# danielbrathwaite/OpenGL-Path-Tracing

Measured on AMD Instinct MI355X. Metric: Mrays/sec + ms/frame @1920×1080, 8 bounces, 1/2/4/8 MI355X, higher is better.
Workload: dtype f32

## Files before the change

### opengl-path-tracing_amd/csrc/pt_cull.h

```cpp
#pragma once

#include "pt_math.h"

namespace ptc {

constexpr float kWindowLo = 0.0001f * 0x1.ff8p-1f;
constexpr float kWindowRay = 0x1.4p-20f;

PT_HD float min_t(float tf, float t) {
#if defined(__HIP_DEVICE_COMPILE__)
    return __builtin_amdgcn_fmed3f(tf, t, -__builtin_huge_valf());
#else
    return fminf(tf, t);
#endif
}

PT_HD void cull_addends(pt::f3 o, pt::f3 rd, const float cm[3], const float ws[3], pt::f3& ol, pt::f3& oh) {
    const pt::f3 ord = pt::mk(-(o.x * rd.x), -(o.y * rd.y), -(o.z * rd.z));
    const float ax = __builtin_fabsf(rd.x), ay = __builtin_fabsf(rd.y), az = __builtin_fabsf(rd.z);
    const pt::f3 e = pt::mk(__builtin_fmaf(cm[0], ax, 0x1p-17f * __builtin_fabsf(ord.x)),
                            __builtin_fmaf(cm[1], ay, 0x1p-17f * __builtin_fabsf(ord.y)),
                            __builtin_fmaf(cm[2], az, 0x1p-17f * __builtin_fabsf(ord.z)));
    const float omax = fmaxf(fmaxf(__builtin_fabsf(o.x), __builtin_fabsf(o.y)), __builtin_fabsf(o.z));
    const float wx = __builtin_fmaf(kWindowRay, omax, ws[0]), wy = __builtin_fmaf(kWindowRay, omax, ws[1]),
                wz = __builtin_fmaf(kWindowRay, omax, ws[2]);
    ol = ord - e;
    oh = ord + pt::mk(__builtin_fmaf(wx, ax, e.x), __builtin_fmaf(wy, ay, e.y), __builtin_fmaf(wz, az, e.z));
}

PT_HD bool cull_hit(float nx, float fx, float ny, float fy, float nz, float fz, pt::f3 rd, pt::f3 ol, pt::f3 oh,
                    float cur_t, float c_lo) {
    const float xn = __builtin_fmaf(nx, rd.x, ol.x), xf = __builtin_fmaf(fx, rd.x, oh.x);
    const float yn = __builtin_fmaf(ny, rd.y, ol.y), yf = __builtin_fmaf(fy, rd.y, oh.y);
    const float zn = __builtin_fmaf(nz, rd.z, ol.z), zf = __builtin_fmaf(fz, rd.z, oh.z);
    const float tn = fmaxf(fmaxf(xn, yn), zn);
    const float tf = fminf(fminf(xf, yf), zf);
    return fmaxf(tn, c_lo) <= min_t(tf, cur_t);
}

inline bool window_slack(const float* bvh, int n_nodes, const float* tris, float ws[3]) {
    const double u = 0x1p-24;
    const float inf = __builtin_huge_valf();
    ws[0] = ws[1] = ws[2] = 0.0f;
    if (n_nodes <= 0) return true;
    double M2 = 0.0;
    for (int q = 0; q < 3; q++) {
        const double m = fmax(fabs((double)bvh[q]), fabs((double)bvh[4 + q]));
        M2 += m * m;
    }
    M2 = sqrt(M2);
    double worst[3] = {0.0, 0.0, 0.0};
    for (int i = 0; i < n_nodes; i++) {
        const float* nd = bvh + 12 * (size_t)i;
        if (!(nd[8] > -1.0f)) continue;
        for (int k = 0; k < 2; k++) {
            const float* t = tris + 16 * (size_t)(int)nd[8 + k];
            const pt::f3 v0 = pt::mk(t[0], t[1], t[2]), v1 = pt::mk(t[4], t[5], t[6]), v2 = pt::mk(t[8], t[9], t[10]);
            const pt::f3 n = pt::normalize(pt::cross(v1 - v0, v2 - v0));
            const float d0 = -pt::dot(n, v0);
            if (!(fabs((double)n.x) + fabs((double)n.y) + fabs((double)n.z) < (double)inf)) continue;
            const double V[3][3] = {{v0.x, v0.y, v0.z}, {v1.x, v1.y, v1.z}, {v2.x, v2.y, v2.z}};
            const double nn[3] = {n.x, n.y, n.z};
            double E1[3], E2[3], L2 = 0.0, rho = 0.0;
            for (int q = 0; q < 3; q++) { E1[q] = V[1][q] - V[0][q]; E2[q] = V[2][q] - V[0][q]; }
            const double N[3] = {E1[1] * E2[2] - E2[1] * E1[2], E1[2] * E2[0] - E2[2] * E1[0], E1[0] * E2[1] - E2[0] * E1[1]};
            const double D = nn[0] * N[0] + nn[1] * N[1] + nn[2] * N[2];
            for (int a = 0; a < 3; a++) {
                const int b = (a + 1) % 3;
                double l2 = 0.0;
                for (int q = 0; q < 3; q++) l2 += (V[b][q] - V[a][q]) * (V[b][q] - V[a][q]);
                L2 = fmax(L2, l2);
                rho = fmax(rho, fabs(nn[0] * V[a][0] + nn[1] * V[a][1] + nn[2] * V[a][2] + (double)d0));
            }
            const double L = sqrt(L2);
            if (!(D > 0.0) || !(L2 <= 0x1p14 * D) || !(rho <= L)) return false;
            const double kappa = L2 / D, z = 1.06 * 0x1p-140 * L / D;
            const double sigma_t = u * (7.2 * M2 + 4.4 * fabs((double)d0)) + 1.14 * rho + 6.5 * z;
            for (int q = 0; q < 3; q++) {
                const double ext = fmax(fmax(V[0][q], V[1][q]), V[2][q]) - fmin(fmin(V[0][q], V[1][q]), V[2][q]);
                worst[q] = fmax(worst[q], 21.4 * u * kappa * ext + 1.021 * sigma_t + 2.0 * z);
            }
        }
    }
    for (int q = 0; q < 3; q++)
        if (!(worst[q] < 0x1p60)) return false;
    for (int q = 0; q < 3; q++) ws[q] = nextafterf((float)(1.25 * worst[q] * (1.0 + 0x1p-20)), inf);
    return true;
}

struct SweepRay { pt::f3 rp, rn, ol, oh; };
PT_HD SweepRay sweep_ray(pt::f3 rd, pt::f3 ol, pt::f3 oh) {
    SweepRay r;
    r.rp = pt::mk(rd.x > 0.0f ? rd.x : 0.0f, rd.y > 0.0f ? rd.y : 0.0f, rd.z > 0.0f ? rd.z : 0.0f);
    r.rn = pt::mk(rd.x > 0.0f ? 0.0f : rd.x, rd.y > 0.0f ? 0.0f : rd.y, rd.z > 0.0f ? 0.0f : rd.z);
    r.ol = ol;
    r.oh = oh;
    return r;
}
PT_HD bool sweep_hit(float lx, float hx, float ly, float hy, float lz, float hz, const SweepRay& r, float t0, float c_lo) {
    const float xn = __builtin_fmaf(lx, r.rp.x, __builtin_fmaf(hx, r.rn.x, r.ol.x));
    const float xf = __builtin_fmaf(hx, r.rp.x, __builtin_fmaf(lx, r.rn.x, r.oh.x));
    const float yn = __builtin_fmaf(ly, r.rp.y, __builtin_fmaf(hy, r.rn.y, r.ol.y));
    const float yf = __builtin_fmaf(hy, r.rp.y, __builtin_fmaf(ly, r.rn.y, r.oh.y));
    const float zn = __builtin_fmaf(lz, r.rp.z, __builtin_fmaf(hz, r.rn.z, r.ol.z));
    const float zf = __builtin_fmaf(hz, r.rp.z, __builtin_fmaf(lz, r.rn.z, r.oh.z));
    const float tn = fmaxf(fmaxf(xn, yn), zn);
    const float tf = fminf(fminf(xf, yf), zf);
    return fmaxf(tn, c_lo) <= min_t(tf, t0);
}
PT_HD unsigned sweep_push(unsigned m, bool hit) {
#if defined(__HIP_DEVICE_COMPILE__) && !defined(PT_SWEEP_NO_ADDC)
    unsigned r;
    const unsigned long long c = __builtin_amdgcn_ballot_w64(hit);
    unsigned long long co;
    asm("v_addc_co_u32 %0, %1, %2, %2, %3" : "=v"(r), "=s"(co) : "v"(m), "s"(c));
    return r;
#else
    return m + m + (hit ? 1u : 0u);
#endif
}
template <class T>
PT_HD unsigned sweep_mask(const SweepRay& r, float t0, float c_lo, T table, int n) {
    unsigned m = 0u;
    for (int k = n - 1; k >= 0; k--) {
        const auto a = table[2 * k], b = table[2 * k + 1];
        m = sweep_push(m, sweep_hit(a.x, a.y, a.z, a.w, b.x, b.y, r, t0, c_lo));
    }
    return m;
}
#if defined(__clang__)
#define PT_SWEEP_UNROLL _Pragma("unroll")
#else
#define PT_SWEEP_UNROLL
#endif
PT_HD void sweep_issue_fence() {
#if defined(__HIP_DEVICE_COMPILE__)
    __builtin_amdgcn_sched_barrier(0);
#endif
}
template <int D> struct SweepChunk { float q[D][6]; };
template <int D, class T>
PT_HD void sweep_chunk_load(SweepChunk<D>& c, T table, int k) {
    PT_SWEEP_UNROLL
    for (int j = 0; j < D; j++) {
        const auto a = table[2 * (k - j)], b = table[2 * (k - j) + 1];
        c.q[j][0] = a.x, c.q[j][1] = a.y, c.q[j][2] = a.z, c.q[j][3] = a.w, c.q[j][4] = b.x, c.q[j][5] = b.y;
    }
}
template <int D>
PT_HD unsigned sweep_chunk_test(unsigned m, const SweepChunk<D>& c, const SweepRay& r, float t0, float c_lo) {
    PT_SWEEP_UNROLL
    for (int j = 0; j < D; j++)
        m = sweep_push(m, sweep_hit(c.q[j][0], c.q[j][1], c.q[j][2], c.q[j][3], c.q[j][4], c.q[j][5], r, t0, c_lo));
    return m;
}
template <int D, class T>
PT_HD unsigned sweep_mask_piped(const SweepRay& r, float t0, float c_lo, T table, int n) {
    static_assert(D >= 1 && D <= 8, "boxes in flight");
    unsigned m = 0u;
    int k = n - 1;
    for (int j = n % D; j > 0; j--, k--) {
        const auto a = table[2 * k], b = table[2 * k + 1];
        m = sweep_push(m, sweep_hit(a.x, a.y, a.z, a.w, b.x, b.y, r, t0, c_lo));
    }
    if (k < 0) return m;
    SweepChunk<D> ca, cb;
    sweep_chunk_load(ca, table, k);
    for (; k >= 3 * D - 1; k -= 2 * D) {
        sweep_chunk_load(cb, table, k - D);
        sweep_issue_fence();
        m = sweep_chunk_test(m, ca, r, t0, c_lo);
        sweep_chunk_load(ca, table, k - 2 * D);
        sweep_issue_fence();
        m = sweep_chunk_test(m, cb, r, t0, c_lo);
    }
    if (k >= 2 * D - 1) {
        sweep_chunk_load(cb, table, k - D);
        m = sweep_chunk_test(m, ca, r, t0, c_lo);
        return sweep_chunk_test(m, cb, r, t0, c_lo);
    }
    return sweep_chunk_test(m, ca, r, t0, c_lo);
}
template <class T>
PT_HD unsigned sweep_mask(pt::f3 rd, pt::f3 ol, pt::f3 oh, float t0, float c_lo, T table, int n) {
    return sweep_mask(sweep_ray(rd, ol, oh), t0, c_lo, table, n);
}
PT_HD bool sweep_root_hit(const float box[6], const SweepRay& r, float t0, float c_lo) {
    return sweep_hit(box[0], box[1], box[2], box[3], box[4], box[5], r, t0, c_lo);
}

}
```

### opengl-path-tracing_amd/csrc/pt_launch_plan.cpp

```cpp
#include "pt_launch_plan.h"

#include "pt_pool.h"

#include "../../include/pt_api.h"

#include <algorithm>
#include <cmath>

namespace ptl {

static int resident_waves(int minw, bool lds) { return minw ? minw : (lds ? 7 : 6); }

static bool lds_staged(const SceneFacts& f, const Tuning& t, const Image& im, const State& s) {
    if (t.variant == 3) return false;
    if (f.lds_bytes <= kLdsSceneSmall) return true;
    return !s.counting && !t.minw && im.rpp == 1 && f.lds_bytes <= kLdsSceneMax;
}

bool cons_walk_on(const SceneFacts& f, const Tuning& t, bool counting) {
    if (!f.walk_nested || t.cons_off || counting) return false;
    const size_t mw = (size_t)resident_waves(t.minw, true);
    const auto blocks = [mw](size_t b) { return b ? std::min(mw, kLdsCu / b) : mw; };
    return blocks(f.lds_bytes_sk) >= blocks(f.lds_bytes);
}

bool window_cull_on(const SceneFacts& f, const Tuning& t, int flags, bool counting) {
    return cons_walk_on(f, t, counting) && !t.win_off && !f.win_bad && !(flags & PT_FLAG_MOLLER_TRUMBORE);
}

bool sweep_on(const SceneFacts& f, const Tuning& t, bool counting) {
    return cons_walk_on(f, t, counting) && f.sweep_ok && !t.sweep_off;
}

static bool wide_walk_on(const SceneFacts& f, const Tuning& t, bool counting) {
    return f.wide_ok && f.scene_fast && !t.wide_off && !counting && t.minw != 8;
}

static int lds_threads(const Tuning& t, const Image& im, const State& s, size_t lds) {
    if (s.counting || t.minw || im.rpp > 1 || !lds) return 256;
    const int per_cu = (int)(kLdsCu / lds);
    int best_k = 1, best = 0;
    for (int k = 1; k <= 4; k++) {
        const int waves = std::min(per_cu, 7 / k) * k;
        if (waves > best) { best = waves; best_k = k; }
    }
    return 256 * best_k;
}

static int plan_group(const SceneFacts& f, const Tuning& t, const Image& im, const State& s, int n_frames) {
    if (t.group_force > 0) return std::min(t.group_force, n_frames);
    const bool lds_scene = lds_staged(f, t, im, s);
    const double lanes = (double)im.n_cu * 4.0 * resident_waves(t.minw, lds_scene) * 64.0;
    const double px = s.adaptive ? (double)im.n_tiles * 64.0 : (double)im.rows_local * im.width;
    const double F = px * n_frames / lanes;
    int g = (int)(std::sqrt(F) * (lds_scene ? 0.416 : 0.19) + 0.5);
    g = std::max(1, std::min(g, lds_scene ? 16 : 4));
    return std::min(g, n_frames);
}

static bool split_mode(const Tuning& t, const State& s, int n_frames, int group) {
    if (s.moments) return true;
    if (group < n_frames) return true;
    return t.group_force == 0 && n_frames <= kShortLaunch;
}

unsigned long long id_limit(const Tuning& t, const Image& im) {
    const unsigned long long pb = (unsigned long long)std::max(256, t.pull_batch);
    const unsigned long long slack = (unsigned long long)im.persist_blocks * 4ull * 2ull * pb;
    return (1ull << 32) - slack - (1ull << 20);
}

int launch_frames(const SceneFacts& f, const Tuning& t, const Image& im, const State& s, int n_frames) {
    const unsigned long long px = (unsigned long long)std::max(im.rows_local, 1) * (unsigned long long)im.width;
    const unsigned long long tiles64 = (unsigned long long)std::max(im.n_tiles, 1) * 64ull;
    const unsigned long long lim = id_limit(t, im);
    int n = n_frames;
    for (;;) {
        const int g = plan_group(f, t, im, s, n);
        if (!split_mode(t, s, n, g)) return n;
        const unsigned long long by_budget = std::max(1ull, (unsigned long long)t.scratch_budget / (px * 12ull));
        const unsigned long long ng = (unsigned long long)((n + g - 1) / g);
        const unsigned long long by_ids = (lim / tiles64) * (unsigned long long)g;
        if (((unsigned long long)n <= by_budget && ng * tiles64 < lim) || n == 1) return n;
        const unsigned long long m = std::min<unsigned long long>({(unsigned long long)n - 1, by_budget, by_ids});
        n = (int)std::max<unsigned long long>(m, 1ull);
    }
}

static KernelKey kernel_key(bool counting, bool lds, bool wide, bool split, int mw, int rpp, int nt, int walk_np) {
    const bool multi = rpp > 1;
    if (wide) {
        if (multi) return {false, false, 6, true, split, false, 256, true};
        if (nt == 512 || nt == 768) return {false, false, 6, false, split, false, nt, true};
        if (nt == 1024) return {false, false, 4, false, split, false, 1024, true};
        return {false, false, mw == 5 || mw == 7 ? mw : 6, false, split, false, 256, true};
    }
    if (nt == 512 || nt == 768) return {false, true, 6, false, split, false, nt, false};
    if (nt > 256) return {false, true, 4, false, split, false, 1024, false};
    if (counting) return {true, lds, 5, multi, split, false, 256, false};
    if (split && mw == 8 && !multi) return {false, lds, 8, false, true, false, 256, false};
    if (split && mw == 7 && !multi) return {false, lds, 7, false, true, lds && walk_np == kPadNodes, 256, false};
    return {false, lds, mw >= 6 ? 6 : 5, multi, split, false, 256, false};
}

static bool common_launch(const SceneFacts& f, const Tuning& t, const Image& im, const LaunchPlan& p) {
    if (t.common_off || t.win_off || f.win_bad || !(p.key == kCommonKey)) return false;
    if (t.minw || t.leaf_thresh || t.shade_thresh || t.trav_floor || im.tile_shift != 0 || !p.cons_walk) return false;
    if (im.flags != 0) return false;
    return f.n_spheres == 1 && f.scene_fast != 0 && f.walk_nested && f.root_child >= 0;
}

LaunchPlan plan_launch(const SceneFacts& f, const Tuning& t, const Image& im, const State& s, int n_frames,
                       bool graph) {
    LaunchPlan p{};
    const bool lds_scene = lds_staged(f, t, im, s);
    p.lds = t.variant == 0 && lds_scene;
    p.wide = !p.lds && wide_walk_on(f, t, s.counting);
    p.cons_walk = cons_walk_on(f, t, s.counting);
    p.leaf_cert = f.leaf_cert_ok && !t.cert_off && !(im.flags & PT_FLAG_MOLLER_TRUMBORE) && p.wide;
    p.leaf_thresh = t.leaf_thresh ? t.leaf_thresh : (lds_scene ? 52 : 20);
    p.shade_thresh = t.shade_thresh ? t.shade_thresh : (lds_scene ? 44 : 24);
    p.trav_floor = t.trav_floor ? t.trav_floor : (lds_scene ? (f.lds_bytes > kLdsSceneSmall ? 8 : 5) : 6);
    p.group = plan_group(f, t, im, s, n_frames);
    p.split = split_mode(t, s, n_frames, p.group);
    const unsigned long long n_groups = (unsigned long long)((n_frames + p.group - 1) / p.group);
    {
        const double waves = (double)im.n_cu * 4.0 * resident_waves(0, lds_scene);
        const double ids = (double)im.n_tiles * (double)n_groups * 64.0;
        const int fit = 16 * (int)(ids / std::max(waves, 1.0) / (8.0 * p.group) / 16.0 + 0.5);
        const int auto_batch = std::max((int)kPullBatch, std::min(256, fit));
        p.pull_batch = t.pull_batch ? t.pull_batch
                                    : (lds_scene && p.group <= 2 ? (p.group == 1 ? 256 : 64) : auto_batch);
    }
    {
        const unsigned long long items = (unsigned long long)im.n_tiles * n_groups;
        p.grp_magic = (n_groups > 1 && items * n_groups < (1ull << 32)) ? (unsigned)(((1ull << 32) + n_groups - 1) / n_groups) : 0u;
    }
    p.overlap = t.overlap_slots > 1 && !graph && !s.counting && !s.adaptive && n_frames <= kShortLaunch && p.split;
    const size_t lds = p.lds ? (p.cons_walk ? f.lds_bytes_sk : f.lds_bytes) : 0;
    const int wide_nt = (p.wide && im.rpp == 1) ? (t.wide_threads ? t.wide_threads : kWideThreadsAuto) : 256;
    p.nt = p.lds ? lds_threads(t, im, s, lds) : (p.wide ? wide_nt : 256);
    p.mw = resident_waves(t.minw, p.lds);
    {
        const unsigned items = (unsigned)im.n_tiles * (unsigned)n_groups;
        const unsigned wpb = (unsigned)p.nt / 64u;
        p.blocks = std::min<unsigned>(im.persist_blocks * 256u / (unsigned)p.nt, std::max(1u, (items + wpb - 1) / wpb));
    }
    if (p.overlap && p.nt == 256) {
        const int bpc = t.overlap_bpc ? t.overlap_bpc
                      : t.overlap_slots >= 3 ? (s.aces_fuse ? std::max(1, p.mw - 2) : 3)
                                             : std::max(1, p.mw - 1);
        p.blocks = std::min<unsigned>(p.blocks, (unsigned)(bpc * im.n_cu));
    }
    p.n_top = p.mw > 6 ? std::min(f.n_top, (int)kLdsCu / p.mw / 32 - 8) : f.n_top;
    const size_t shade_bytes = (size_t)(3 * f.n_mats + 2 * f.n_spheres) * 16;
    p.shade_lds = shade_bytes <= 4096;
    const size_t shade_lds_bytes = p.shade_lds ? shade_bytes : 0;
    if (p.wide) {
        const size_t blocks_cu = wide_nt == 1024 ? 1
                               : (wide_nt == 256 ? (size_t)(im.rpp > 1 ? 6 : std::min(std::max(p.mw, 5), 7))
                                                 : (size_t)(6 * 256 / wide_nt));
        p.wide_top = (int)std::min<size_t>({(size_t)f.n_wide, (size_t)kWideTopMax,
                                            (kLdsCu / blocks_cu - shade_lds_bytes - 1024) / 48});
    }
    p.dyn_lds_bytes = p.lds ? lds : (p.wide ? (size_t)p.wide_top * 48 : (size_t)p.n_top * 32) + shade_lds_bytes;
    p.key = kernel_key(s.counting, p.lds, p.wide, p.split, p.mw, im.rpp, p.nt, f.walk_np);
    p.common = !s.adaptive && common_launch(f, t, im, p);
    p.sweep = p.lds && p.nt == 256 && sweep_on(f, t, s.counting);
    if (p.sweep && !t.shade_thresh) p.shade_thresh = kSweepShadeThresh;
    {
        p.pool_paths = kPoolPaths, p.pool_nt = kPoolThreads;
        const int wpb = kPoolThreads / 64;
        const size_t scene = (size_t)(4 * f.n_slots + 3 * f.n_mats + 2 * f.n_spheres + 2 * f.n_leaves) * 16;
        p.pool_lds_bytes = ptpool::block_bytes(kPoolPaths, wpb, scene);
        const int full_cu = 4 * kPoolWaves / wpb;
        const int per_cu = (int)std::min<size_t>(kLdsCu / (p.pool_lds_bytes + 1024), (size_t)full_cu);
        p.pool = kPoolDefault && !t.pool_off && p.common && p.sweep && !p.overlap && per_cu >= 1 && per_cu == full_cu &&
                 ptpool::pack_ok(im.width, im.rows_local, n_frames, 0, f.n_slots, f.n_spheres);
        const unsigned long long paths = (unsigned long long)im.n_tiles * n_groups * 64ull, per_block = (unsigned long long)(kPoolPaths * wpb);
        p.pool_blocks = (unsigned)std::min<unsigned long long>((unsigned long long)std::max(per_cu, 1) * (unsigned long long)std::max(im.n_cu, 1),
                                                               std::max(1ull, (paths + per_block - 1) / per_block));
    }
    if (p.split) {
        p.accum_long = n_frames > kShortLaunch;
        p.accum_moments = s.moments;
        p.aces_out = s.aces_fuse && !graph;
        const long long px = (long long)im.rows_local * im.width, per_block = 256 * (p.accum_long ? kAccumPixLong : kAccumPix);
        p.accum_blocks = (unsigned)((px + per_block - 1) / per_block);
    }
    return p;
}

size_t scratch_bytes(const LaunchPlan& plan, const Image& im, int n_frames) {
    if (!plan.split) return 0;
    return (size_t)std::max(im.rows_local, 1) * (size_t)im.width * (size_t)n_frames * 3 * sizeof(float);
}

}
```

### opengl-path-tracing_amd/csrc/pt_render_phase.h

```cpp
namespace {

typedef float v4f __attribute__((ext_vector_type(4)));
typedef __attribute__((address_space(3))) const v4f lds_v4f;
typedef __attribute__((address_space(4))) const v4f const_v4f;

template <bool LDS>
__device__ __forceinline__ float4 tri_quad(const SceneView& S, int slot, int k) {
#ifdef PT_DIAG_TRIS_GLOBAL
    return S.tris[4 * slot + k];
#else
    return LDS ? S.tris[slot + k * S.tp] : S.tris[4 * slot + k];
#endif
}

using pt::in_guard;
using pt::in_range_abs;

using pt::win_open;
using pt::win_closed;

__device__ __forceinline__ int rank_in(unsigned long long m) {
    return (int)__builtin_amdgcn_mbcnt_hi((unsigned)(m >> 32), __builtin_amdgcn_mbcnt_lo((unsigned)m, 0u));
}

template <bool COMMON, bool SWEEP = false>
struct LaunchFacts {
    const KParams& p;
    __device__ __forceinline__ bool sweep() const { return COMMON ? SWEEP : p.sweep != 0; }
    __device__ __forceinline__ int mode() const { return COMMON ? 1 : p.mode; }
    __device__ __forceinline__ int flags() const { return COMMON ? 0 : p.flags; }
    __device__ __forceinline__ bool cons_walk() const { return COMMON || p.cons_walk != 0; }
    __device__ __forceinline__ bool scene_fast() const { return COMMON || p.scene_fast != 0; }
    __device__ __forceinline__ float win_lo() const { return COMMON ? ptc::kWindowLo : p.win_lo; }
    __device__ __forceinline__ int n_spheres() const { return COMMON ? 1 : p.sc.n_spheres; }
    __device__ __forceinline__ int tile_shift() const { return COMMON ? 0 : p.tile_shift; }
    __device__ __forceinline__ bool tile_perm() const { return COMMON || p.tile_perm != nullptr; }
    __device__ __forceinline__ bool tile_cost() const { return COMMON || p.tile_cost != nullptr; }
    __device__ __forceinline__ bool inside(int cx, int cy) const { return COMMON || ((cx < p.x_limit) & (cy < p.y_limit)); }
};

__device__ __forceinline__ void stage_tris_chain_order(float4* dst, const KParams& p, int T, int nthreads) {
    for (int i = threadIdx.x; i < 4 * T; i += nthreads) {
        const int slot = i >> 2, c = __float_as_int(p.sweep_tab[2 * (slot >> 1) + 1].w);
        dst[(i & 3) * T + 2 * c + (slot & 1)] = p.sc.tris[i];
    }
}

template <bool LDS, class Facts>
__device__ __forceinline__ bool shade_segment(const Facts& F, const KParams& p, const SceneView& S, bool hit, int hprim,
                                              float t, f3& o, f3& d, f3& inc, f3& col, uint32_t& state, int& bounce,
                                              f3& rgb) {
    bool finished = false;
    rgb = inc;
    if (hit && pt::length_gt_001(col)) {
        const f3 hitp = o + d * t;
        f3 normal;
        int mat;
        if (hprim >= 0) {
            const float4 nq = tri_quad<LDS>(S, hprim, 0);
            normal = mk(nq.x, nq.y, nq.z);
            mat = __float_as_int(tri_quad<LDS>(S, hprim, 2).w);
        } else {
            const int si = -2 - hprim;
            float4 s0 = S.spheres[2 * si];
            normal = pt::normalize(hitp - mk(s0.x, s0.y, s0.z));
            mat = __float_as_int(S.spheres[2 * si + 1].x);
        }
        if (pt::dot(normal, d) > 0.0f) normal = normal * -1.0f;
        if (F.mode() == 2) {
            rgb = (normal + mk(1, 1, 1)) * 0.5f;
            finished = true;
        } else if (F.mode() == 4) {
            float s = pt::length(hitp - o);
            float dist = 1.0f - pt::fsqrt(s + 1.0f) / (s + 1.0f);
            float q = dist * dist;
            rgb = mk(q, q, q);
            finished = true;
        } else {
            o = hitp;
            f3 diffuse = pt::normalize(normal + pt::random_unit_vector(state));
            float kk = 2.0f * pt::dot(normal, d);
            f3 specular = pt::normalize(d - normal * kk);
            float4 m0 = S.mats[3 * mat], m1 = S.mats[3 * mat + 1], m2 = S.mats[3 * mat + 2];
            if (F.mode() == 3) {
                rgb = mk(m0.x, m0.y, m0.z);
                finished = true;
            } else {
                float is_spec = (m1.w > pt::random01(state)) ? 1.0f : 0.0f;
                d = pt::mix(diffuse, specular, m0.w * is_spec);
                inc = inc + mk(m1.x, m1.y, m1.z) * col;
                col = col * pt::mix(mk(m0.x, m0.y, m0.z), mk(m2.x, m2.y, m2.z), is_spec);
                bounce++;
                if (bounce > p.max_bounce) {
                    rgb = inc;
                    finished = true;
                }
            }
        }
    } else {
        f3 env = mk(0, 0, 0);
        if (!(F.flags() & PT_FLAG_NO_SKY)) {
            f3 dir = pt::normalize(d);
            float tt = 0.5f * (dir.z + 1.0f);
            float omt = 1.0f - tt;
            env = mk(omt * 1.0f + tt * 0.5f, omt * 1.0f + tt * 0.7f, omt * 1.0f + tt * 1.0f);
        }
        rgb = inc + env * col;
        finished = true;
    }
    return finished;
}

struct QueueIds { unsigned id, qnext, qend; };
template <bool SPLIT>
__device__ __forceinline__ QueueIds queue_ids(const KParams& p, bool want, unsigned long long m, unsigned qnext,
                                              unsigned qend) {
    const unsigned need = (unsigned)__popcll(m);
    const unsigned rank = (unsigned)rank_in(m);
    const int leader = __ffsll((long long)m) - 1;
    unsigned id;
    if (SPLIT && qend - qnext >= need) {
        id = qnext + rank;
        qnext += need;
    } else {
        const unsigned avail = SPLIT ? qend - qnext : 0u;
        const unsigned take = SPLIT ? max(need - avail, (unsigned)p.pull_batch) : need;
        unsigned base = 0;
        if (want && rank == 0u) base = atomicAdd(p.work_counter, take);
        base = (unsigned)__builtin_amdgcn_readlane((int)base, leader);
        id = rank < avail ? qnext + rank : base + (rank - avail);
        if (SPLIT) {
            qnext = base + (need - avail);
            qend = base + take;
        }
    }
    const QueueIds q = {id, qnext, qend};
    return q;
}

template <class Facts>
__device__ __forceinline__ void camera_ray(const Facts& F, const KParams& p, f3 cpos, f3 cfwd, f3 cright, f3 cup, int lx,
                                           int y, int k, int r, uint32_t& state, f3& o, f3& d, f3& inc, f3& col,
                                           int& bounce) {
    if (r == 0) state = pt::seed(lx, y, p.frame_first + k);
    float ax = 0.0f, ay = 0.0f;
    if (!(F.flags() & PT_FLAG_NO_AA)) {
        ax = pt::random01(state);
        ay = pt::random01(state);
    }
    float u = pt::div_mk((float)lx + ax, p.fW, p.rW) - 0.5f;
    float v = pt::div_mk((float)y + ay, p.fH, p.rH) - 0.5f;
    d = pt::normalize((cfwd + cright * u) + cup * v);
    o = cpos;
    inc = mk(0, 0, 0);
    col = mk(1, 1, 1);
    bounce = 0;
}

template <class Facts>
__device__ __forceinline__ bool seg_in_guard(const Facts& F, f3 o, f3 d) {
    return F.scene_fast() & in_guard(o.x, 0x1p-40f, 0x1p60f) & in_guard(o.y, 0x1p-40f, 0x1p60f) &
           in_guard(o.z, 0x1p-40f, 0x1p60f) & in_range_abs(d.x, 0x1p-20f, 2.0f) &
           in_range_abs(d.y, 0x1p-20f, 2.0f) & in_range_abs(d.z, 0x1p-20f, 2.0f);
}

__device__ __forceinline__ float sphere_t(const SceneView& S, int si, f3 o, f3 d) {
    float4 s0 = S.spheres[2 * si];
    f3 oc = o - mk(s0.x, s0.y, s0.z);
    float a = pt::dot(d, d);
    float half_b = pt::dot(oc, d);
    float cq = pt::dot(oc, oc) - s0.w;
    float disc = half_b * half_b - a * cq;
    return disc < 0.0f ? -1.0f : (-half_b - pt::sqrt_g(disc)) / a;
}

template <int DEPTH = 0, class Table>
__device__ __forceinline__ unsigned sweep_candidates(const KParams& p, const SceneView& S, Table table,
                                                     bool on, f3 o, f3 rd, float t) {
    unsigned cand = 0u;
    if (on) {
        f3 ol, oh;
        ptc::cull_addends(o, rd, S.cm, S.ws, ol, oh);
        const ptc::SweepRay sr = ptc::sweep_ray(rd, ol, oh);
        bool in = true;
        if (p.sweep_root) in = ptc::sweep_root_hit(p.root_box, sr, t, S.clo);
        if (in) cand = DEPTH > 0 ? ptc::sweep_mask_piped<(DEPTH > 0 ? DEPTH : 1)>(sr, t, S.clo, table, p.n_sweep)
                                 : ptc::sweep_mask(sr, t, S.clo, table, p.n_sweep);
    }
    return cand;
}

struct LeafChoice { bool c1, c2; };
__device__ __forceinline__ LeafChoice leaf_choice(float h1, float h2, float t) {
    const bool c1 = win_open(h1, t) & ((h1 < h2) | (h2 < 0.0001f));
    const bool c2 = !c1 & win_open(h2, t);
    const LeafChoice r = {c1, c2};
    return r;
}

}
```

### opengl-path-tracing_amd/csrc/pt_render_pool.h

```cpp
#ifndef PT_POOL_SWEEP_DEPTH
#define PT_POOL_SWEEP_DEPTH 2
#endif
#ifndef PT_POOL_SWEEP_LDS
#define PT_POOL_SWEEP_LDS 1
#endif
namespace {

__device__ __forceinline__ void pool_cold_walk(const KParams& p, const SceneView& S, f3 o, f3 d, float& t, int& hprim) {
    int w = 0;
    while (w >= 0) {
        const float4 lo = p.sc.nodes[2 * w], hi = p.sc.nodes[2 * w + 1];
        const int a = __float_as_int(hi.z), b = __float_as_int(hi.w);
        if (!slab(lo, hi, o, d, t)) { w = b; continue; }
        if (a >= 0) { w = a; continue; }
        const int q = (~a) >> 2;
        const int s0 = 2 * __float_as_int(p.sweep_tab[2 * q + 1].w);
        const bool cop = __float_as_int(tri_quad<true>(S, s0 + 1, 1).w) != 0;
        const float4 nda = tri_quad<true>(S, s0, 0);
        const float4 ndb = cop ? nda : tri_quad<true>(S, s0 + 1, 0);
        const float ta = tri_plane(nda, o, d);
        const float tb = cop ? ta : tri_plane(ndb, o, d);
        bool oka = false, okb = false, ca = false, cb = false;
        if (win_open(ta, t)) oka = tri_edges_at<true, false>(S, s0, mk(nda.x, nda.y, nda.z), o + d * ta, false, 0.0f, ca);
        if (win_closed(tb, t)) okb = tri_edges_at<true, false>(S, s0 + 1, mk(ndb.x, ndb.y, ndb.z), o + d * tb, false, 0.0f, cb);
        const float h1 = oka ? ta : -1.0f, h2 = okb ? tb : -1.0f;
        const LeafChoice lc = leaf_choice(h1, h2, t);
        if (lc.c1 | lc.c2) {
            t = lc.c1 ? h1 : h2;
            hprim = s0 + (lc.c1 ? 0 : 1);
        }
        w = b;
    }
}

__device__ __forceinline__ void pool_pass_fence() {
    __builtin_amdgcn_fence(__ATOMIC_RELEASE, "wavefront");
    __builtin_amdgcn_wave_barrier();
    __builtin_amdgcn_fence(__ATOMIC_ACQUIRE, "wavefront");
}

template <int NT, int P, int MINW>
__global__ __launch_bounds__(NT, MINW) void k_render_pool(KParams p) {
    static_assert(P >= 64 && P <= ptpool::kMaxPaths && P % 4 == 0, "one-byte list entries in a 16-byte padded array");
    using namespace ptpool;
    const LaunchFacts<true, true> F{p};
    const const_v4f* const sweep_tab = (const const_v4f*)(size_t)p.sweep_tab;
    (void)sweep_tab;
    resolve_frames(p);
    extern __shared__ float4 lds[];
    const int T = p.n_slots, nt = 4 * T, nm = 3 * p.n_mats, ns = 2, nb = 2 * p.n_sweep;
    stage_tris_chain_order(lds, p, T, NT);
    for (int i = threadIdx.x; i < nm; i += NT) lds[nt + i] = p.sc.mats[i];
    for (int i = threadIdx.x; i < ns; i += NT) lds[nt + nm + i] = p.sc.spheres[i];
    for (int i = threadIdx.x; i < nb; i += NT) lds[nt + nm + ns + i] = p.sweep_tab[i];
    const int scene_q = nt + nm + ns + nb;
    const int lane = (int)(threadIdx.x & 63u);
    float4* const pool = lds + scene_q + (int)(threadIdx.x >> 6) * (wave_bytes(P) / 16);
    unsigned char* const list = (unsigned char*)(pool + kChunks * P);
    for (int i = lane; i < P; i += kLanes) {
        pool[quad_of(kChunkO, i, P)] = make_float4(0, 0, 0, -1.0f);
        pool[quad_of(kChunkD, i, P)] = make_float4(0, 0, 1, 0);
        pool[quad_of(kChunkInc, i, P)] = make_float4(0, 0, 0, __uint_as_float(pack_hit(-1, -1)));
        pool[quad_of(kChunkCol, i, P)] = make_float4(1, 1, 1, 0);
        pool[quad_of(kChunkItem, i, P)] = make_float4(__uint_as_float(kNoItem), 0, 0, 0);
        list[i] = (unsigned char)i;
    }
    __syncthreads();
    SceneView S;
    S.nodes = nullptr;
    S.tris = lds;
    S.mats = lds + nt;
    S.spheres = lds + nt + nm;
    const float4* const boxes = lds + nt + nm + ns;
    S.np = 0;
    S.tp = T;
    S.cm[0] = p.cons_m[0], S.cm[1] = p.cons_m[1], S.cm[2] = p.cons_m[2];
    S.ws[0] = p.win_slack[0], S.ws[1] = p.win_slack[1], S.ws[2] = p.win_slack[2];
    S.clo = ptc::kWindowLo;
    const f3 cpos = mk(p.cam[0], p.cam[1], p.cam[2]), cfwd = mk(p.cam[3], p.cam[4], p.cam[5]);
    const f3 cright = mk(p.cam[6], p.cam[7], p.cam[8]), cup = mk(p.cam[9], p.cam[10], p.cam[11]);
    const int tiles_x = (p.W + 7) >> 3;
    const unsigned n_groups = (unsigned)((p.n_frames + p.group - 1) / p.group);
    const unsigned total_ids = p.queue_tiles * n_groups * 64u;
    unsigned qnext = 0, qend = 0;
    Lists L = {P, 0};
    while (L.nS + L.nL > 0) {
        const int phase = choose(L), n = take(L, phase);
        const bool on = lane < n;
        int idx = 0;
        if (on) idx = list[pop_index(L, phase, n, lane, P)];
        drop(L, phase, n);
        bool to_shade = false, to_leaf = false;
        if (phase == kShade) {
            const float4 c0 = pool[quad_of(kChunkO, idx, P)], c1 = pool[quad_of(kChunkD, idx, P)];
            const float4 c2 = pool[quad_of(kChunkInc, idx, P)], c3 = pool[quad_of(kChunkCol, idx, P)];
            const float4 c4 = pool[quad_of(kChunkItem, idx, P)];
            f3 o = mk(c0.x, c0.y, c0.z), d = mk(c1.x, c1.y, c1.z), inc = mk(c2.x, c2.y, c2.z), col = mk(c3.x, c3.y, c3.z);
            float t = c0.w;
            unsigned bi = __float_as_uint(c1.w);
            int hprim = hit_hprim(__float_as_uint(c2.w)), bounce = hit_bounce(__float_as_uint(c2.w));
            uint32_t state = __float_as_uint(c3.w);
            unsigned xy = __float_as_uint(c4.x);
            int aidx = __float_as_int(c4.y);
            int k = k_k(__float_as_uint(c4.z)), kend = k_kend(__float_as_uint(c4.z));
            unsigned pcost = cost_of(__float_as_uint(c4.w));
            bool report = cost_report(__float_as_uint(c4.w));
            bool retired = false;
            if (on && !(t < 0.0f)) {
                const bool hit = hprim != -1;
                pcost++;
                f3 rgb;
                const bool finished = shade_segment<true>(F, p, S, hit, hprim, t, o, d, inc, col, state, bounce, rgb);
                if (finished) {
                    bounce = -1;
                    const f3 px = (mk(0, 0, 0) + rgb) / 1.0f;
                    nt_store3(p.rgb + 3 * ((size_t)k * (size_t)(p.rows_local * p.W) + (size_t)aidx), px);
                    k++;
                }
                t = -1.0f;
            }
            if (on & (bounce < 0) & (xy != kNoItem) & (k >= kend)) {
                if (report) atomicAdd(&p.tile_cost[(xy_crow(xy) >> 3) * tiles_x + (xy_lx(xy) >> 3)], pcost);
                xy = kNoItem;
            }
            const bool want = on && xy == kNoItem;
            const unsigned long long m = __ballot(want);
            if (m) {
                const QueueIds qi = queue_ids<true>(p, want, m, qnext, qend);
                const unsigned id = qi.id;
                qnext = qi.qnext, qend = qi.qend;
                if (want) {
                    if (id >= total_ids) {
                        retired = true;
                    } else {
                        const unsigned item = id >> 6, w = id & 63u;
                        const unsigned tile = p.grp_magic ? __umulhi(item, p.grp_magic) : item;
                        const int g = (int)(item - tile * n_groups);
                        const unsigned pk = p.tile_perm[tile];
                        const int tx = (int)(pk & 0xffffu), ty = (int)(pk >> 16);
                        const int cx = tx * 8 + (int)(w & 7u);
                        const int crow = ty * 8 + (int)(w >> 3);
                        if ((cx < p.W) & (crow < p.rows_local)) {
                            xy = pack_xy(cx, crow);
                            aidx = crow * p.W + cx;
                            report = (w & 0x1bu) == 0u;
                            pcost = 0;
                            k = g * p.group;
                            kend = min(k + p.group, p.n_frames);
                            bounce = -1;
                        }
                    }
                }
            }
            if (on && xy != kNoItem) {
                const int lx = xy_lx(xy), y = p.row0 + xy_crow(xy) * p.row_stride;
                if (bounce < 0) camera_ray(F, p, cpos, cfwd, cright, cup, lx, y, k, 0, state, o, d, inc, col, bounce);
                const bool fast_seg = seg_in_guard(F, o, d);
                const f3 rd = fast_seg ? mk(pt::rcp_fast(d.x), pt::rcp_fast(d.y), pt::rcp_fast(d.z)) : mk(0, 0, 0);
                t = __builtin_huge_valf();
                hprim = -1;
                {
                    const float ht = sphere_t(S, 0, o, d);
                    if (win_open(ht, t)) {
                        t = ht;
                        hprim = -2;
                    }
                }
                const bool walk = !ray_has_nan(o, d);
#if PT_POOL_SWEEP_DEPTH > 0 && PT_POOL_SWEEP_LDS
                const unsigned cand = sweep_candidates<PT_POOL_SWEEP_DEPTH>(p, S, boxes, walk & fast_seg, o, rd, t);
#else
                const unsigned cand = sweep_candidates<PT_POOL_SWEEP_DEPTH>(p, S, sweep_tab, walk & fast_seg, o, rd, t);
#endif
                const bool cold = walk & !fast_seg;
                if (__any(cold)) {
                    if (cold) pool_cold_walk(p, S, o, d, t, hprim);
                }
                bi = cand;
                to_leaf = cand != 0u;
            }
            to_shade = on & !retired & !to_leaf;
            if (on) {
                pool[quad_of(kChunkO, idx, P)] = make_float4(o.x, o.y, o.z, t);
                pool[quad_of(kChunkD, idx, P)] = make_float4(d.x, d.y, d.z, __uint_as_float(bi));
                pool[quad_of(kChunkInc, idx, P)] = make_float4(inc.x, inc.y, inc.z, __uint_as_float(pack_hit(hprim, bounce)));
                pool[quad_of(kChunkCol, idx, P)] = make_float4(col.x, col.y, col.z, __uint_as_float(state));
                pool[quad_of(kChunkItem, idx, P)] = make_float4(__uint_as_float(xy), __int_as_float(aidx),
                                                                __uint_as_float(pack_k(k, kend)),
                                                                __uint_as_float(pack_cost(pcost, report)));
            }
        } else {
            const float4 c0 = pool[quad_of(kChunkO, idx, P)], c1 = pool[quad_of(kChunkD, idx, P)];
            float* const hw = (float*)&pool[quad_of(kChunkInc, idx, P)] + 3;
            const unsigned hb = __float_as_uint(*hw);
            const f3 o = mk(c0.x, c0.y, c0.z), d = mk(c1.x, c1.y, c1.z);
            float t = c0.w;
            unsigned bi = __float_as_uint(c1.w);
            const bool at = on;
            int s0 = 0, lp = 0;
            bool cop = false;
            float4 nd0 = make_float4(0, 0, 0, 0);
            if (at) {
                lp = __ffs((int)bi) - 1;
                s0 = 2 * lp;
                cop = __float_as_int(tri_quad<true>(S, s0 + 1, 1).w) != 0;
                nd0 = tri_quad<true>(S, s0, 0);
            }
            float h1 = -1.0f, h2 = -1.0f;
            bool ca = false, cb = false;
            leaf_pair_tests<true, false>(S, at, s0, nd0, cop, o, d, t, p.compact_max, h1, h2, false, ca, cb);
            bool c1h = false, c2h = false;
            if (at) {
                const LeafChoice lc = leaf_choice(h1, h2, t);
                c1h = lc.c1, c2h = lc.c2;
            }
            const bool chk = at & (c1h | c2h);
            if (__any(chk)) {
                if (chk) {
                    const f3 rd = mk(pt::rcp_fast(d.x), pt::rcp_fast(d.y), pt::rcp_fast(d.z));
                    if (!slab_fast(boxes[2 * lp], boxes[2 * lp + 1], o, d, rd, t)) c1h = c2h = false;
                }
            }
            if (at) {
                int hprim = hit_hprim(hb);
                if (c1h | c2h) {
                    t = c1h ? h1 : h2;
                    hprim = s0 + (c1h ? 0 : 1);
                }
                bi &= bi - 1u;
                to_leaf = bi != 0u;
                to_shade = bi == 0u;
                ((float*)&pool[quad_of(kChunkO, idx, P)])[3] = t;
                ((float*)&pool[quad_of(kChunkD, idx, P)])[3] = __uint_as_float(bi);
                *hw = __uint_as_float(with_hprim(hb, hprim));
            }
        }
        const unsigned long long mS = __ballot(to_shade), mL = __ballot(to_leaf);
        if (to_shade) list[push_index(L, kShade, rank_in(mS), P)] = (unsigned char)idx;
        if (to_leaf) list[push_index(L, kLeaf, rank_in(mL), P)] = (unsigned char)idx;
        grow(L, kShade, __popcll(mS));
        grow(L, kLeaf, __popcll(mL));
        pool_pass_fence();
    }
}

}
```

Measured before the change: 37010.

## Store leaf boxes as sign-ordered per-axis pairs to drop select math in sweep

Leaf bounding boxes in LDS are restaged as three float4 per leaf, each holding (lo,hi,hi,lo) for one axis. Each ray picks a float2 offset per axis from its direction sign, so the sweep reads near/far directly and uses the plain cull_hit test instead of the rp/rn two-FMA formulation. This cuts ALU work per box test but grows the LDS box table from 2 to 3 quads per leaf, which may lower occupancy. Loads become three 8-byte reads per box rather than two 16-byte reads.

Result: faster. 38590, median of 6 (+4.3%).

```diff
diff --git a/opengl-path-tracing_amd/csrc/pt_cull.h b/opengl-path-tracing_amd/csrc/pt_cull.h
--- a/opengl-path-tracing_amd/csrc/pt_cull.h
+++ b/opengl-path-tracing_amd/csrc/pt_cull.h
@@ -185,6 +185,61 @@
 PT_HD unsigned sweep_mask(pt::f3 rd, pt::f3 ol, pt::f3 oh, float t0, float c_lo, T table, int n) {
     return sweep_mask(sweep_ray(rd, ol, oh), t0, c_lo, table, n);
 }
+constexpr int kSignedQuads = 3;
+constexpr int kSignedPairs = 2 * kSignedQuads;
+template <class Q>
+PT_HD void sweep_signed_quad(const Q& a, const Q& b, int axis, float q[4]) {
+    const float lo = axis == 0 ? a.x : (axis == 1 ? a.z : b.x), hi = axis == 0 ? a.y : (axis == 1 ? a.w : b.y);
+    q[0] = lo, q[1] = hi, q[2] = hi, q[3] = lo;
+}
+PT_HD int sweep_signed_pair(float rd_axis, int axis) { return 2 * axis + (rd_axis > 0.0f ? 0 : 1); }
+PT_HD bool sweep_hit_signed(float xn, float xf, float yn, float yf, float zn, float zf, pt::f3 rd, pt::f3 ol, pt::f3 oh,
+                            float t0, float c_lo) {
+    return cull_hit(xn, xf, yn, yf, zn, zf, rd, ol, oh, t0, c_lo);
+}
+template <int D, class P>
+PT_HD void sweep_signed_load(SweepChunk<D>& c, P px, P py, P pz, int k) {
+    PT_SWEEP_UNROLL
+    for (int j = 0; j < D; j++) {
+        const auto x = px[kSignedPairs * (k - j)], y = py[kSignedPairs * (k - j)], z = pz[kSignedPairs * (k - j)];
+        c.q[j][0] = x.x, c.q[j][1] = x.y, c.q[j][2] = y.x, c.q[j][3] = y.y, c.q[j][4] = z.x, c.q[j][5] = z.y;
+    }
+}
+template <int D>
+PT_HD unsigned sweep_signed_test(unsigned m, const SweepChunk<D>& c, pt::f3 rd, pt::f3 ol, pt::f3 oh, float t0, float c_lo) {
+    PT_SWEEP_UNROLL
+    for (int j = 0; j < D; j++)
+        m = sweep_push(m, sweep_hit_signed(c.q[j][0], c.q[j][1], c.q[j][2], c.q[j][3], c.q[j][4], c.q[j][5], rd, ol, oh, t0, c_lo));
+    return m;
+}
+template <int D, class P>
+PT_HD unsigned sweep_mask_signed_piped(pt::f3 rd, pt::f3 ol, pt::f3 oh, float t0, float c_lo, P px, P py, P pz, int n) {
+    static_assert(D >= 1 && D <= 8, "boxes in flight");
+    unsigned m = 0u;
+    int k = n - 1;
+    for (int j = n % D; j > 0; j--, k--) {
+        SweepChunk<1> c;
+        sweep_signed_load(c, px, py, pz, k);
+        m = sweep_signed_test(m, c, rd, ol, oh, t0, c_lo);
+    }
+    if (k < 0) return m;
+    SweepChunk<D> ca, cb;
+    sweep_signed_load(ca, px, py, pz, k);
+    for (; k >= 3 * D - 1; k -= 2 * D) {
+        sweep_signed_load(cb, px, py, pz, k - D);
+        sweep_issue_fence();
+        m = sweep_signed_test(m, ca, rd, ol, oh, t0, c_lo);
+        sweep_signed_load(ca, px, py, pz, k - 2 * D);
+        sweep_issue_fence();
+        m = sweep_signed_test(m, cb, rd, ol, oh, t0, c_lo);
+    }
+    if (k >= 2 * D - 1) {
+        sweep_signed_load(cb, px, py, pz, k - D);
+        m = sweep_signed_test(m, ca, rd, ol, oh, t0, c_lo);
+        return sweep_signed_test(m, cb, rd, ol, oh, t0, c_lo);
+    }
+    return sweep_signed_test(m, ca, rd, ol, oh, t0, c_lo);
+}
 PT_HD bool sweep_root_hit(const float box[6], const SweepRay& r, float t0, float c_lo) {
     return sweep_hit(box[0], box[1], box[2], box[3], box[4], box[5], r, t0, c_lo);
 }
diff --git a/opengl-path-tracing_amd/csrc/pt_launch_plan.cpp b/opengl-path-tracing_amd/csrc/pt_launch_plan.cpp
--- a/opengl-path-tracing_amd/csrc/pt_launch_plan.cpp
+++ b/opengl-path-tracing_amd/csrc/pt_launch_plan.cpp
@@ -171,7 +171,7 @@
     {
         p.pool_paths = kPoolPaths, p.pool_nt = kPoolThreads;
         const int wpb = kPoolThreads / 64;
-        const size_t scene = (size_t)(4 * f.n_slots + 3 * f.n_mats + 2 * f.n_spheres + 2 * f.n_leaves) * 16;
+        const size_t scene = (size_t)(4 * f.n_slots + 3 * f.n_mats + 2 * f.n_spheres + 3 * f.n_leaves) * 16;
         p.pool_lds_bytes = ptpool::block_bytes(kPoolPaths, wpb, scene);
         const int full_cu = 4 * kPoolWaves / wpb;
         const int per_cu = (int)std::min<size_t>(kLdsCu / (p.pool_lds_bytes + 1024), (size_t)full_cu);
diff --git a/opengl-path-tracing_amd/csrc/pt_render_phase.h b/opengl-path-tracing_amd/csrc/pt_render_phase.h
--- a/opengl-path-tracing_amd/csrc/pt_render_phase.h
+++ b/opengl-path-tracing_amd/csrc/pt_render_phase.h
@@ -190,6 +190,22 @@
     return cand;
 }
 
+template <int DEPTH>
+__device__ __forceinline__ unsigned sweep_candidates_signed(const KParams& p, const SceneView& S, const float2* pairs,
+                                                            bool on, f3 o, f3 rd, float t) {
+    unsigned cand = 0u;
+    if (on) {
+        f3 ol, oh;
+        ptc::cull_addends(o, rd, S.cm, S.ws, ol, oh);
+        bool in = true;
+        if (p.sweep_root) in = ptc::sweep_root_hit(p.root_box, ptc::sweep_ray(rd, ol, oh), t, S.clo);
+        if (in) cand = ptc::sweep_mask_signed_piped<DEPTH>(rd, ol, oh, t, S.clo, pairs + ptc::sweep_signed_pair(rd.x, 0),
+                                                           pairs + ptc::sweep_signed_pair(rd.y, 1),
+                                                           pairs + ptc::sweep_signed_pair(rd.z, 2), p.n_sweep);
+    }
+    return cand;
+}
+
 struct LeafChoice { bool c1, c2; };
 __device__ __forceinline__ LeafChoice leaf_choice(float h1, float h2, float t) {
     const bool c1 = win_open(h1, t) & ((h1 < h2) | (h2 < 0.0001f));
diff --git a/opengl-path-tracing_amd/csrc/pt_render_pool.h b/opengl-path-tracing_amd/csrc/pt_render_pool.h
--- a/opengl-path-tracing_amd/csrc/pt_render_pool.h
+++ b/opengl-path-tracing_amd/csrc/pt_render_pool.h
@@ -4,6 +4,10 @@
 #ifndef PT_POOL_SWEEP_LDS
 #define PT_POOL_SWEEP_LDS 1
 #endif
+#ifndef PT_POOL_SWEEP_SIGNED
+#define PT_POOL_SWEEP_SIGNED 1
+#endif
+#define PT_POOL_SIGNED_ON (PT_POOL_SWEEP_SIGNED && PT_POOL_SWEEP_LDS && PT_POOL_SWEEP_DEPTH > 0)
 namespace {
 
 __device__ __forceinline__ void pool_cold_walk(const KParams& p, const SceneView& S, f3 o, f3 d, float& t, int& hprim) {
@@ -48,11 +52,22 @@
     (void)sweep_tab;
     resolve_frames(p);
     extern __shared__ float4 lds[];
-    const int T = p.n_slots, nt = 4 * T, nm = 3 * p.n_mats, ns = 2, nb = 2 * p.n_sweep;
+    const int T = p.n_slots, nt = 4 * T, nm = 3 * p.n_mats, ns = 2, nb = ptc::kSignedQuads * p.n_sweep;
     stage_tris_chain_order(lds, p, T, NT);
     for (int i = threadIdx.x; i < nm; i += NT) lds[nt + i] = p.sc.mats[i];
     for (int i = threadIdx.x; i < ns; i += NT) lds[nt + nm + i] = p.sc.spheres[i];
-    for (int i = threadIdx.x; i < nb; i += NT) lds[nt + nm + ns + i] = p.sweep_tab[i];
+#if PT_POOL_SIGNED_ON
+    for (int leaf = threadIdx.x; leaf < p.n_sweep; leaf += NT) {
+        const float4 a = p.sweep_tab[2 * leaf], b = p.sweep_tab[2 * leaf + 1];
+        for (int axis = 0; axis < ptc::kSignedQuads; axis++) {
+            float q[4];
+            ptc::sweep_signed_quad(a, b, axis, q);
+            lds[nt + nm + ns + ptc::kSignedQuads * leaf + axis] = make_float4(q[0], q[1], q[2], q[3]);
+        }
+    }
+#else
+    for (int i = threadIdx.x; i < 2 * p.n_sweep; i += NT) lds[nt + nm + ns + i] = p.sweep_tab[i];
+#endif
     const int scene_q = nt + nm + ns + nb;
     const int lane = (int)(threadIdx.x & 63u);
     float4* const pool = lds + scene_q + (int)(threadIdx.x >> 6) * (wave_bytes(P) / 16);
@@ -72,6 +87,8 @@
     S.mats = lds + nt;
     S.spheres = lds + nt + nm;
     const float4* const boxes = lds + nt + nm + ns;
+    const float2* const signed_pairs = (const float2*)boxes;
+    (void)signed_pairs;
     S.np = 0;
     S.tp = T;
     S.cm[0] = p.cons_m[0], S.cm[1] = p.cons_m[1], S.cm[2] = p.cons_m[2];
@@ -167,7 +184,9 @@
                     }
                 }
                 const bool walk = !ray_has_nan(o, d);
-#if PT_POOL_SWEEP_DEPTH > 0 && PT_POOL_SWEEP_LDS
+#if PT_POOL_SIGNED_ON
+                const unsigned cand = sweep_candidates_signed<PT_POOL_SWEEP_DEPTH>(p, S, signed_pairs, walk & fast_seg, o, rd, t);
+#elif PT_POOL_SWEEP_DEPTH > 0 && PT_POOL_SWEEP_LDS
                 const unsigned cand = sweep_candidates<PT_POOL_SWEEP_DEPTH>(p, S, boxes, walk & fast_seg, o, rd, t);
 #else
                 const unsigned cand = sweep_candidates<PT_POOL_SWEEP_DEPTH>(p, S, sweep_tab, walk & fast_seg, o, rd, t);
@@ -218,7 +237,13 @@
             if (__any(chk)) {
                 if (chk) {
                     const f3 rd = mk(pt::rcp_fast(d.x), pt::rcp_fast(d.y), pt::rcp_fast(d.z));
+#if PT_POOL_SIGNED_ON
+                    const float2 bx = signed_pairs[ptc::kSignedPairs * lp], by = signed_pairs[ptc::kSignedPairs * lp + 2];
+                    const float2 bz = signed_pairs[ptc::kSignedPairs * lp + 4];
+                    if (!slab_fast(make_float4(bx.x, bx.y, by.x, by.y), make_float4(bz.x, bz.y, 0, 0), o, d, rd, t)) c1h = c2h = false;
+#else
                     if (!slab_fast(boxes[2 * lp], boxes[2 * lp + 1], o, d, rd, t)) c1h = c2h = false;
+#endif
                 }
             }
             if (at) {
```
